# ParBLiSS/kmerhash

Measured on AMD Instinct MI355X. Metric: kmer_inserts_plus_finds_per_sec, higher is better.
Workload: dtype u64

## Files before the change

### kmerhash_amd/csrc/kh_kernels.h

```cpp
#pragma once
#include <hip/hip_runtime.h>
#include <stdint.h>
#include "../../include/kmerhash_amd/kh_hash.h"

#define KH_LB 11
#define KH_L (1u << KH_LB)
#define KH_HS 4096u
#define KH_CHUNK_THREADS 512
#ifndef KH_PART_THREADS
#define KH_PART_THREADS 512
#define KH_PART_MAXPER 4
#endif
#ifndef KH_PART_ITEMS
#define KH_PART_ITEMS 16
#endif
#define KH_PART_TILE (KH_PART_THREADS * KH_PART_ITEMS)
#ifndef KH_PART_STAGE
#define KH_PART_STAGE 4096
#endif
#define KH_NONE 0xFFFFFFFFFFFFFFFFull
#define KH_EMPTY_KEY 0xFFFFFFFFFFFFFFFFull

enum { KHK_RH = 0, KHK_LP = 1 };
enum { KH_FLAG_PROBE_OVERFLOW = 0, KH_FLAG_REGION_OVERFLOW = 1, KH_FLAG_COUNT_OVERFLOW = 2, KH_FLAG_INTERNAL = 3, KH_FLAG_FUSE_INVALID = 4, KH_NFLAGS = 8 };

template <int KIND> __device__ __forceinline__ bool kh_is_empty(uint32_t b) { return KIND == KHK_RH ? (b == 0x00u) : (b == 0x40u); }
template <int KIND> __device__ __forceinline__ bool kh_is_occupied(uint32_t b) { return KIND == KHK_RH ? (b >= 0x80u) : (b < 0x40u); }

struct __align__(16) KhSlot { uint64_t key; uint32_t val; uint32_t info; };
#define KH_INFO_ERASE_MARK 0x100u
struct KhSlots {
  KhSlot* s;
  uint64_t cap;
};
__device__ __forceinline__ uint4 kh_slot_ld(const KhSlot* p) { return *reinterpret_cast<const uint4*>(p); }
__device__ __forceinline__ void kh_slot_st(KhSlot* p, uint64_t key, uint32_t val, uint32_t info) {
  uint4 w; w.x = (uint32_t)key; w.y = (uint32_t)(key >> 32); w.z = val; w.w = info;
  *reinterpret_cast<uint4*>(p) = w;
}
__device__ __forceinline__ uint64_t kh_slot_key(const uint4& w) { return (uint64_t)w.x | ((uint64_t)w.y << 32); }
template <int KIND> __device__ __forceinline__ uint32_t kh_empty_info() { return KIND == KHK_RH ? 0x00u : 0x40u; }

// ... 435 lines not shown
  const KhTile* tiles;
  const uint32_t* ntiles_dev;
  uint32_t ntiles;
  KhSeed seed;
  uint32_t PB;
  uint32_t shift;
  uint32_t nb;
  uint32_t* counts;
  unsigned long long* cursor;
  ulonglong2* orec;
  uint64_t slot;
  uint64_t dump;
  uint32_t* overflow;
  int xcd_swizzle;
  uint64_t slot_in; const unsigned long long* cur_in; uint32_t tps;
};

__device__ __forceinline__ uint32_t kh_part_q(uint64_t h, uint32_t PB) {
  if (PB == 0) return 0;
  uint32_t p = (uint32_t)(h >> KH_LB) & ((1u << PB) - 1u);
  return __brev(p) >> (32 - PB);
}

__device__ __forceinline__ KhTile kh_get_tile(const KhPartParams& P, uint32_t t) {
  if (P.tiles) return P.tiles[t];
  KhTile d;
  d.beg = (uint64_t)t * KH_PART_TILE;
  uint64_t rem = P.n - d.beg;
  d.len = rem < KH_PART_TILE ? (uint32_t)rem : KH_PART_TILE;
  d.seg = 0;
  return d;
}

template <int HASH, bool REC8 = false>
__global__ __launch_bounds__(KH_PART_THREADS) void k_part_hist(KhPartParams P) {
  extern __shared__ __align__(16) uint32_t kh_dyn_smem[];
  uint32_t* hist = kh_dyn_smem;
  const uint32_t tid = threadIdx.x, nb = P.nb;
  const uint32_t ntiles = P.tiles ? *P.ntiles_dev : P.ntiles;
  for (uint32_t i = tid; i < nb; i += KH_PART_THREADS) hist[i] = 0;
  __syncthreads();
  const uint32_t tpb = (ntiles + gridDim.x - 1) / gridDim.x;
  const uint32_t t0 = blockIdx.x * tpb;
  const uint32_t t1 = (t0 + tpb < ntiles) ? t0 + tpb : ntiles;
  uint32_t cur_seg = 0xFFFFFFFFu;
  for (uint32_t t = t0; t < t1; ++t) {
    KhTile d = kh_get_tile(P, t);
    if (d.seg != cur_seg) {
      if (cur_seg != 0xFFFFFFFFu) {
        __syncthreads();
        for (uint32_t i = tid; i < nb; i += KH_PART_THREADS) {
          uint32_t c = hist[i];
// ... 8 lines not shown
                              : *reinterpret_cast<const uint64_t*>(P.kbase + (d.beg + i) * P.kstride);
      uint32_t q = kh_part_q(kh_hash64<HASH>(key, P.seed), P.PB);
      atomicAdd(&hist[(q >> P.shift) & (nb - 1)], 1u);
    }
  }
  __syncthreads();
  if (cur_seg != 0xFFFFFFFFu)
    for (uint32_t i = tid; i < nb; i += KH_PART_THREADS) {
      uint32_t c = hist[i];
      if (c) atomicAdd(&P.counts[(uint64_t)cur_seg * nb + i], c);
    }
}

__device__ __forceinline__ void kh_rec_set(ulonglong2& r, uint64_t key, unsigned long long iv) { r = make_ulonglong2(key, iv); }
__device__ __forceinline__ void kh_rec_set(KhRec12& r, uint64_t key, unsigned long long iv) { r.klo = (uint32_t)key; r.khi = (uint32_t)(key >> 32); r.val = (uint32_t)iv; }
__device__ __forceinline__ void kh_rec_get(const ulonglong2& r, uint64_t& key, unsigned long long& iv) { key = r.x; iv = r.y; }
__device__ __forceinline__ void kh_rec_get(const KhRec12& r, uint64_t& key, unsigned long long& iv) { key = r.klo | ((uint64_t)r.khi << 32); iv = r.val; }
struct KhRec8 { uint64_t key; };
__device__ __forceinline__ void kh_rec_set(KhRec8& r, uint64_t key, unsigned long long) { r.key = key; }
__device__ __forceinline__ void kh_rec_get(const KhRec8& r, uint64_t& key, unsigned long long& iv) { key = r.key; iv = 0; }
template <int RK> struct KhRecOf { typedef ulonglong2 type; };
template <> struct KhRecOf<1> { typedef KhRec12 type; };
template <> struct KhRecOf<2> { typedef KhRec8 type; };
#ifdef KH_PART_OCC3
#define KH_PART_LB(RK) __launch_bounds__(KH_PART_THREADS, (RK) ? 6 : 4)
#define KH_PART_STAGE_OF(RK) ((RK) == 1 ? 3072u : (uint32_t)KH_PART_STAGE)
#else
#define KH_PART_LB(RK) __launch_bounds__(KH_PART_THREADS)
#define KH_PART_STAGE_OF(RK) ((uint32_t)KH_PART_STAGE)
#endif
template <int HASH, int RK>
__global__ KH_PART_LB(RK) void k_part_scatter(KhPartParams P) {
  constexpr bool R12 = RK != 0;
  constexpr uint32_t STAGE = KH_PART_STAGE_OF(RK);
  typedef typename KhRecOf<RK>::type Rec;
  extern __shared__ __align__(16) uint32_t kh_dyn_smem[];
  __shared__ Rec lrec[STAGE];
  __shared__ uint16_t ld[STAGE];
  __shared__ uint32_t wtot[KH_PART_THREADS / 64];
  const uint32_t nb = P.nb;
  uint32_t* hist = kh_dyn_smem;
  uint32_t* loff = kh_dyn_smem + nb;
  unsigned long long* gbase = reinterpret_cast<unsigned long long*>(kh_dyn_smem + 2 * ((nb + 1u) & ~1u));
  const uint32_t tid = threadIdx.x, lane = tid & 63, wid = tid >> 6;
  const uint32_t ntiles = P.tiles ? *P.ntiles_dev : P.ntiles;
  if (blockIdx.x >= ntiles) return;
  uint32_t tile = blockIdx.x;
  if (P.xcd_swizzle && (tile | 63u) < ntiles) {
    const uint32_t x = tile & 7u, j = (tile >> 3) & 7u;
    tile = (tile & ~63u) + x * 8u + j;
  }
  KhTile d;
  uint32_t last;
  unsigned long long fill_end = 0;
  if (P.slot_in) {
    const uint32_t seg = tile / P.tps, k = tile - seg * P.tps;
    fill_end = P.cur_in[seg];
    d.seg = seg; d.beg = (uint64_t)seg * P.slot_in + (uint64_t)k * KH_PART_TILE; d.len = 0;
    const uint64_t room = P.slot_in - (uint64_t)k * KH_PART_TILE;
    last = (room < KH_PART_TILE ? (uint32_t)room : KH_PART_TILE) - 1u;
  } else {
    d = kh_get_tile(P, tile);
    if (d.len == 0) return;
    last = d.len - 1u;
  }
  for (uint32_t i = tid; i < nb; i += KH_PART_THREADS) hist[i] = 0;
  uint64_t key[KH_PART_ITEMS];
  unsigned long long iv[KH_PART_ITEMS];
  uint32_t dr[KH_PART_ITEMS];
  if (P.rec_in) {
    const Rec* src = reinterpret_cast<const Rec*>(P.rec_in) + d.beg;
    Rec rr[KH_PART_ITEMS];
#pragma unroll
    for (int j = 0; j < KH_PART_ITEMS; ++j) { const uint32_t i = tid + j * KH_PART_THREADS; rr[j] = src[i < last ? i : last]; }
#pragma unroll
    for (int j = 0; j < KH_PART_ITEMS; ++j) kh_rec_get(rr[j], key[j], iv[j]);
  } else {
    const char* kb = P.kbase + d.beg * P.kstride;
#pragma unroll
    for (int j = 0; j < KH_PART_ITEMS; ++j) {
      const uint32_t i = tid + j * KH_PART_THREADS, ic = i < last ? i : last;
      key[j] = *reinterpret_cast<const uint64_t*>(kb + (uint64_t)ic * P.kstride);
    }
    if (P.vbase) {
      const char* vb = P.vbase + d.beg * P.vstride;
#pragma unroll
      for (int j = 0; j < KH_PART_ITEMS; ++j) {
        const uint32_t i = tid + j * KH_PART_THREADS, ic = i < last ? i : last;
        iv[j] = *reinterpret_cast<const uint32_t*>(vb + (uint64_t)ic * P.vstride);
      }
    } else {
#pragma unroll
      for (int j = 0; j < KH_PART_ITEMS; ++j) iv[j] = P.vconst;
    }
    if (!R12) {
      const uint64_t pos0 = P.idx_base + d.beg;
#pragma unroll
      for (int j = 0; j < KH_PART_ITEMS; ++j) iv[j] |= (unsigned long long)(pos0 + tid + j * KH_PART_THREADS) << 32;
    }
  }
  if (P.slot_in) {
    const uint64_t sbeg = (uint64_t)d.seg * P.slot_in;
    uint64_t fill = fill_end - sbeg;
    if (fill > P.slot_in) fill = P.slot_in;
    const uint64_t off = d.beg - sbeg;
    if (off == (uint64_t)(P.tps - 1u) * KH_PART_TILE && fill > (uint64_t)P.tps * KH_PART_TILE && tid == 0) *P.overflow = 1u;
    d.len = fill > off ? (fill - off < KH_PART_TILE ? (uint32_t)(fill - off) : KH_PART_TILE) : 0u;
    if (d.len == 0) return;
  }
  __syncthreads();
#pragma unroll
  for (int j = 0; j < KH_PART_ITEMS; ++j) {
    const uint32_t i = tid + j * KH_PART_THREADS;
    const uint32_t q = kh_part_q(kh_hash64<HASH>(key[j], P.seed), P.PB);
    const uint32_t dg = (q >> P.shift) & (nb - 1);
    dr[j] = dg << 16;
    if (i < d.len) dr[j] |= atomicAdd(&hist[dg], 1u);
  }
  __syncthreads();
  const uint32_t per = (nb + KH_PART_THREADS - 1) / KH_PART_THREADS;
  uint32_t mine = 0;
  for (uint32_t k = 0; k < per; ++k) { uint32_t b = tid * per + k; if (b < nb) mine += hist[b]; }
  uint32_t incl = mine;
  for (int off = 1; off < 64; off <<= 1) {
    uint32_t o = __shfl_up(incl, off, 64);
    if (lane >= (uint32_t)off) incl += o;
  }
  if (lane == 63) wtot[wid] = incl;
  __syncthreads();
  uint32_t run = incl - mine;
  for (uint32_t w = 0; w < wid; ++w) run += wtot[w];
  unsigned long long gres[KH_PART_MAXPER];
#pragma unroll
  for (uint32_t k = 0; k < KH_PART_MAXPER; ++k) {
    gres[k] = 0;
    const uint32_t b = tid * per + k;
    if (k < per && b < nb) {
      const uint32_t c = hist[b];
      loff[b] = run;
      run += c;
      if (c) {
        unsigned long long g = atomicAdd(&P.cursor[(uint64_t)d.seg * nb + b], (unsigned long long)c);
        if (P.slot && g + c > ((uint64_t)d.seg * nb + b + 1) * P.slot) { *P.overflow = 1u; g = P.dump + loff[b]; }
        gres[k] = g;
      }
    }
  }
  __syncthreads();
  for (uint32_t r0 = 0; r0 < d.len; r0 += STAGE) {
    if (r0) __syncthreads();
#pragma unroll
    for (int j = 0; j < KH_PART_ITEMS; ++j) {
      uint32_t i = tid + j * KH_PART_THREADS;
      if (i < d.len) {
        const uint32_t dg = dr[j] >> 16;
        const uint32_t s = loff[dg] + (dr[j] & 0xFFFFu) - r0;
        if (s < STAGE) { kh_rec_set(lrec[s], key[j], iv[j]); ld[s] = (uint16_t)dg; }
      }
    }
    if (r0 == 0) {
#pragma unroll
      for (uint32_t k = 0; k < KH_PART_MAXPER; ++k) {
        const uint32_t b = tid * per + k;
        if (k < per && b < nb) gbase[b] = gres[k];
      }
    }
    __syncthreads();
    const uint32_t rl = d.len - r0 < STAGE ? d.len - r0 : STAGE;
    for (uint32_t s = tid; s < rl; s += KH_PART_THREADS) {
      const uint32_t dd = ld[s];
      const uint64_t pos = gbase[dd] + (r0 + s - loff[dd]);
      reinterpret_cast<Rec*>(P.orec)[pos] = lrec[s];
    }
  }
}

#define KH_FULLHIST_THREADS 1024
template <int HASH>
__global__ __launch_bounds__(KH_FULLHIST_THREADS) void k_part_hist_full(const char* __restrict__ kbase, uint32_t kstride, uint64_t n, KhSeed seed,
                                                                         uint32_t PB, uint32_t slice, uint32_t slice_bits,
                                                                         uint32_t* __restrict__ counts ) {
  extern __shared__ __align__(16) uint32_t kh_dyn_smem[];
  const uint32_t lb = PB - slice_bits;
  const uint32_t words = lb ? (1u << (lb - 1)) : 1u;
  const uint32_t lmask = (1u << lb) - 1u;
  for (uint32_t i = threadIdx.x; i < words; i += KH_FULLHIST_THREADS) kh_dyn_smem[i] = 0;
  __syncthreads();
  const uint64_t per = (n + gridDim.x - 1) / gridDim.x;
  const uint64_t b0 = (uint64_t)blockIdx.x * per;
  const uint64_t b1 = b0 + per < n ? b0 + per : n;
  for (uint64_t i0 = b0 + threadIdx.x; i0 < b1; i0 += 8 * KH_FULLHIST_THREADS) {
    uint64_t key[8];
// ... 2806 lines not shown
```

### kmerhash_amd/csrc/kmerhash_amd.hip

```cpp
#include "kh_kernels.h"
#include "kh_kernels_wide.h"
#include "../../include/kmerhash_amd.h"

#include <string>
#include <vector>
#include <cstdio>
#include <cstring>
#include <algorithm>
#include <cmath>
#include <cstdlib>

#include <map>
#include <memory>
#include <mutex>
#include <unordered_map>

#define KH_VERSION_STR "kmerhash_amd 0.1 (gfx950)"

namespace {
struct DevPool {
  std::mutex m;
  std::multimap<size_t, void*> free_;
  std::unordered_map<void*, size_t> size_of;
  size_t cached = 0;
// ... 470 lines not shown
  { kh_status ps = arena_prepare(t, ws_rebuild(n)); if (ps != KH_OK) return ps; }
  return rebuild(t, n, nullptr, nullptr, nullptr, nullptr, 0, false, t->lsize);
}
kh_status do_reserve(kh_table* t, uint64_t n) {
  if (n > t->max_load) return do_rehash(t, static_cast<uint64_t>(static_cast<float>(n) / t->max_lf));
  return KH_OK;
}

struct Partitioned {
  ulonglong2* rec;
  uint64_t* part_off;
  uint32_t PB, nparts;
  ulonglong2* spare;
  uint64_t slot;
  const unsigned long long* cursor;
  uint32_t* overflow;
  int rec12;
};
inline uint64_t slack_slot(double mean, double vf = 1.0) { return (uint64_t)(mean + 7.0 * std::sqrt(mean * vf) + 16.0); }
const bool g_disable_slack = getenv("KH_DISABLE_SLACK_PARTITION") != nullptr;
const int g_xcd_swizzle = getenv("KH_DISABLE_XCD_SWIZZLE") ? 0 : 1;
inline uint64_t part_buffer_records(uint64_t n, uint32_t PB, bool allow_slack, double vf = 1.0) {
  if (!allow_slack || g_disable_slack || PB <= 11 || n < (uint64_t(256) << PB)) return n;
  return (slack_slot((double)n / (double)(uint64_t(1) << PB), vf) << PB) + KH_PART_TILE;
}

kh_status partition_batch(kh_table* t, const char* kbase, uint32_t kstride, const char* vbase, uint32_t vstride,
                          uint32_t vconst, uint64_t n, uint64_t idx_base, uint32_t PB, ulonglong2* tmp, ulonglong2* fin, Partitioned& out,
                          bool allow_slack = false, int rec12 = 0, const SlackShared* shared = nullptr, bool force_slack = false, double vf = 1.0) {
  const uint32_t nparts = 1u << PB;
  out.slot = 0; out.cursor = nullptr; out.overflow = nullptr; out.rec12 = 0;
  if (shared || force_slack || part_buffer_records(n, PB, allow_slack, vf) != n) {
    const uint32_t B1 = (PB + 1) / 2, B2 = PB - B1, nb1 = 1u << B1, nb2 = 1u << B2;
    const uint64_t slot = shared ? shared->slot : slack_slot((double)n / (double)nparts, vf);
    const uint64_t slot1 = shared ? slack_slot((double)n / (double)nb1) : slot * nb2;
    unsigned long long *cur1, *cur2; uint64_t* starts; uint32_t* ovf;
    TAKE(cur1, unsigned long long, nb1);
    if (shared) { cur2 = shared->cur2; starts = shared->starts; ovf = shared->ovf; }
    else { TAKE(cur2, unsigned long long, nparts); TAKE(starts, uint64_t, (size_t)nparts + 1); TAKE(ovf, uint32_t, 1); }
    const double mean1 = (double)n / (double)nb1;
    const uint64_t fill_cap = std::min<uint64_t>(slot1, (uint64_t)(mean1 + 9.0 * std::sqrt(mean1 * vf) + 16.0));
    const uint32_t tps = (uint32_t)((fill_cap + KH_PART_TILE - 1) / KH_PART_TILE);
    const uint32_t max_tiles = nb1 * tps;
    if (shared) hipLaunchKernelGGL(k_init_cursors, dim3((nb1 + 255) / 256), dim3(256), 0, t->stream, cur1, (uint64_t*)nullptr, (uint64_t)nb1, slot1);
    else hipLaunchKernelGGL(k_init_cursors2, dim3((nparts + 256) / 256), dim3(256), 0, t->stream, cur1, (uint64_t)nb1, slot1, cur2, starts, (uint64_t)nparts, slot, ovf);
    KhPartParams P;
    memset(&P, 0, sizeof(P));
    P.idx_base = idx_base;
    P.xcd_swizzle = g_xcd_swizzle;
    P.kbase = kbase; P.kstride = kstride; P.vbase = vbase; P.vstride = vstride; P.vconst = vconst; P.n = n;
    P.ntiles = (uint32_t)((n + KH_PART_TILE - 1) / KH_PART_TILE);
    P.seed = t->seed; P.PB = PB; P.shift = B2; P.nb = nb1; P.cursor = cur1; P.orec = tmp; P.slot = slot1; P.overflow = ovf; P.dump = slot1 * nb1;
    { Launch L(t, "k_part_scatter");
      if (rec12 == 1) { KH_SWITCH_HASH(t->hash, hipLaunchKernelGGL((k_part_scatter<HASH, 1>), dim3(P.ntiles), dim3(KH_PART_THREADS), ((nb1 + 1u) & ~1u) * 8 + nb1 * 8, t->stream, P)); }
      else if (rec12 == 2) { KH_SWITCH_HASH(t->hash, hipLaunchKernelGGL((k_part_scatter<HASH, 2>), dim3(P.ntiles), dim3(KH_PART_THREADS), ((nb1 + 1u) & ~1u) * 8 + nb1 * 8, t->stream, P)); }
      else { KH_SWITCH_HASH(t->hash, hipLaunchKernelGGL((k_part_scatter<HASH, 0>), dim3(P.ntiles), dim3(KH_PART_THREADS), ((nb1 + 1u) & ~1u) * 8 + nb1 * 8, t->stream, P)); } }
    KhPartParams Q = P;
    Q.kbase = nullptr; Q.kstride = 0; Q.vbase = nullptr; Q.vstride = 0; Q.rec_in = tmp;
    Q.tiles = nullptr; Q.ntiles_dev = nullptr; Q.ntiles = max_tiles; Q.slot_in = slot1; Q.cur_in = cur1; Q.tps = tps;
    Q.shift = 0; Q.nb = nb2; Q.cursor = cur2; Q.orec = fin; Q.slot = slot; Q.dump = slot * nparts;
    { Launch L(t, "k_part_scatter");
      if (rec12 == 1) { KH_SWITCH_HASH(t->hash, hipLaunchKernelGGL((k_part_scatter<HASH, 1>), dim3(max_tiles), dim3(KH_PART_THREADS), ((nb2 + 1u) & ~1u) * 8 + nb2 * 8, t->stream, Q)); }
      else if (rec12 == 2) { KH_SWITCH_HASH(t->hash, hipLaunchKernelGGL((k_part_scatter<HASH, 2>), dim3(max_tiles), dim3(KH_PART_THREADS), ((nb2 + 1u) & ~1u) * 8 + nb2 * 8, t->stream, Q)); }
      else { KH_SWITCH_HASH(t->hash, hipLaunchKernelGGL((k_part_scatter<HASH, 0>), dim3(max_tiles), dim3(KH_PART_THREADS), ((nb2 + 1u) & ~1u) * 8 + nb2 * 8, t->stream, Q)); } }
    HIPCHK(hipGetLastError());
    out.rec = fin; out.part_off = starts; out.PB = PB; out.nparts = nparts; out.spare = tmp;
    out.slot = slot; out.cursor = cur2; out.overflow = ovf; out.rec12 = rec12;
    return KH_OK;
  }
  if (rec12 == 1) return fail(t, KH_ERR_HIP, "internal: record kind not available with exact offsets");
  ulonglong2* ar = nullptr; ulonglong2* br = fin;
  const uint32_t B1 = PB <= 11 ? PB : (PB + 1) / 2, B2 = PB - B1;
  const uint32_t nb1 = 1u << B1, nb2 = 1u << B2;
  ar = B2 ? tmp : fin;
  uint32_t* counts1; uint64_t* off1; unsigned long long* cur1;
  TAKE(counts1, uint32_t, nb1); TAKE(off1, uint64_t, nb1 + 1); TAKE(cur1, unsigned long long, nb1);
  KhPartParams P;
  memset(&P, 0, sizeof(P));
  P.idx_base = idx_base;
  P.xcd_swizzle = g_xcd_swizzle;
  P.kbase = kbase; P.kstride = kstride; P.vbase = vbase; P.vstride = vstride; P.vconst = vconst; P.rec_in = nullptr; P.n = n;
  P.tiles = nullptr; P.ntiles_dev = nullptr; P.ntiles = (uint32_t)((n + KH_PART_TILE - 1) / KH_PART_TILE);
  P.seed = t->seed; P.PB = PB; P.shift = B2; P.nb = nb1; P.counts = counts1; P.cursor = cur1;
  P.orec = ar;
  KhTile* tiles = nullptr; uint32_t* ntiles_dev = nullptr; uint32_t* counts2 = nullptr; uint64_t* off2 = nullptr; unsigned long long* cur2 = nullptr;
// ... 82 lines not shown
kh_status insert_finish(kh_table* t, KhSrcSet S, uint64_t n, uint32_t PB, uint64_t cap_u, int mode, uint64_t forced_cap,
                        ulonglong2* spare, uint64_t* n_new_out, uint64_t list_cap = 0);

inline bool fused_build_applies(const kh_table* t, uint64_t cap_u, uint32_t PB) {
  return t->lsize == 0 && cap_u >= 2 * (uint64_t)KH_L && t->max_lf <= 0.9f && PB == log2u(cap_u >> KH_LB) && !g_disable_fused;
}
inline bool nodup_build_applies(const kh_table* t, uint64_t cap_u, uint32_t PB, int mode) {
  return fused_build_applies(t, cap_u, PB) && t->batch_nodup && mode != INS_UPDATE && !getenv("KH_DISABLE_NODUP");
}

kh_status insert_core(kh_table* t, const char* kbase, uint32_t kstride, const char* vbase, uint32_t vstride,
                      uint64_t n, int mode, uint64_t forced_cap, uint64_t* n_new_out) {
  *n_new_out = 0;
  if (n == 0) return KH_OK;
  const uint64_t cap_u = forced_cap ? forced_cap : capacity_after(t, t->cur.cap, t->lsize, n, n, n - 1);
  const uint32_t PB = cap_u > KH_L ? log2u(cap_u >> KH_LB) : 0u;
  if (PB > 22) return fail(t, KH_ERR_UNSUPPORTED, "batch would need more than 2^22 partitions");
  const size_t keep_blk = t->blk, keep_off = t->off;
  int first_attempt = 0;
  bool dup_heavy = false;
  double vf = 1.0;
  if (part_buffer_records(n, PB, true) != n) {
    unsigned long long* sset; uint32_t* dups;
    TAKE(sset, unsigned long long, KH_SAMPLE_SET); TAKE(dups, uint32_t, 1);
    HIPCHK(hipMemsetAsync(sset, 0, sizeof(unsigned long long) * KH_SAMPLE_SET, t->stream));
    HIPCHK(hipMemsetAsync(dups, 0, 4, t->stream));
    { Launch L(t, "k_sample_dups");
      hipLaunchKernelGGL(k_sample_dups, dim3(KH_SAMPLE_N / 256), dim3(256), 0, t->stream, kbase, kstride, n, sset, dups); }
    HIPCHK(hipMemcpyAsync(t->hpin + 31, dups, 4, hipMemcpyDeviceToHost, t->stream));
    HIPCHK(hipStreamSynchronize(t->stream));
    const uint32_t dsample = (uint32_t)t->hpin[31];
    if (dsample >= 1u) {
      dup_heavy = true;
      const double d_ub = (double)dsample + 3.0 * std::sqrt((double)dsample) + 3.0;
      const double f = 1.0 + 2.0 * (double)n * d_ub / ((double)KH_SAMPLE_N * (double)KH_SAMPLE_N);
      const double mean = (double)n / (double)(uint64_t(1) << PB);
      if (!getenv("KH_DISABLE_DUP_SLACK") && (double)slack_slot(mean, f) <= 2.0 * mean) vf = f;
      else first_attempt = 1;
    }
    t->batch_nodup = dsample == 0u;
    t->blk = keep_blk; t->off = keep_off;
  } else first_attempt = 1;
  for (int attempt = first_attempt; attempt < 2; ++attempt) {
    const bool slack = attempt == 0;
    const uint64_t m = part_buffer_records(n, PB, slack, vf);
    if (!slack && attempt == 1) { t->blk = keep_blk; t->off = keep_off; }
    const bool rec12 = slack && t->batch_nodup && nodup_build_applies(t, cap_u, PB, mode);
    const bool rec8 = !rec12 && dup_heavy && mode == INS_PLUS && vbase == nullptr && !getenv("KH_DISABLE_REC8");
    const int kind = rec12 ? 1 : rec8 ? 2 : 0;
// ... 529 lines not shown
    }
    st = launch_find(t, out_pairs ? KH_FIND_PAIRS : KH_FIND_COMPACT, q, n, out_pairs ? nullptr : cv, nullptr, out_pairs ? nullptr : ck,
                     out_pairs ? cp : nullptr, &hits_dev);
    if (st != KH_OK) return st;
    HIPCHK(hipMemcpyAsync(t->hpin, hits_dev, 8, hipMemcpyDeviceToHost, t->stream));
    HIPCHK(hipStreamSynchronize(t->stream));
    hits = t->hpin[0];
    if (host && hits) {
      if (out_pairs) { HIPCHK(hipMemcpyAsync(out_pairs, cp, hits * 16, hipMemcpyDeviceToHost, t->stream)); HIPCHK(hipStreamSynchronize(t->stream)); }
      else { st = copy_compacted(t, hits, ck, cv, out_ckeys, out_cvals); if (st != KH_OK) return st; }
    }
  }
  if (n_found) *n_found = hits;
  return KH_OK;
}

kh_status erase_core(kh_table* t, const void* keys, uint64_t n, kh_mem where, uint64_t* n_erased) {
  *n_erased = 0;
  if (t->ins.active) return refuse_streaming(t);
  if (n == 0) return KH_OK;
  if (!keys) return fail(t, KH_ERR_INVALID, "null keys");
  HIPCHK(hipSetDevice(t->device));
  { kh_status ps = inplace_ok(t, n) ? arena_prepare(t, n * 8 + ws_inplace(t, n))
                                    : arena_prepare(t, n * 8 + 2 * 8 * ((slack_slot((double)n / (double)std::max<uint64_t>(1, t->cur.cap >> KH_LB)) * std::max<uint64_t>(1, t->cur.cap >> KH_LB)) + KH_PART_TILE + n) +
                                                       ws_rebuild(t->cur.cap) + (t->cur.cap > KH_L ? (t->cur.cap >> KH_LB) : 1) * 96 + (n / KH_PART_TILE + 4096) * 16 + (size_t(2) << 20));
    if (ps != KH_OK) return ps; }
  const uint64_t* q;
  kh_status st = stage_in<uint64_t>(t, keys, n, where, &q);
  if (st != KH_OK) return st;
  if (t->kind == KHK_RH && n <= KH_SMALL_N && t->lsize > 0 && !g_disable_small) {
    uint64_t ne = 0; uint32_t done = 0;
    st = small_batch(t, reinterpret_cast<const char*>(q), 8, nullptr, 0, 0, (uint32_t)n, KH_SMALL_ERASE, &ne, &done);
    if (st != KH_OK) return st;
    t->lsize -= ne;
    *n_erased = ne;
    return KH_OK;
  }
  if (inplace_ok(t, n)) {
    KhInplaceParams src;
    memset(&src, 0, sizeof(src));
    src.in_k = q; src.n = n;
    IpResult* res = nullptr;
    st = inplace_passes<KH_IP_ERASE>(t, src, n, &res);
    if (st != KH_OK) return st;
    HIPCHK(hipMemcpyAsync(t->hpin, &res->done, 8, hipMemcpyDeviceToHost, t->stream));
    HIPCHK(hipStreamSynchronize(t->stream));
    t->lsize -= t->hpin[0];
    *n_erased = t->hpin[0];
    return KH_OK;
  }
  const uint32_t PBe = t->cur.cap > KH_L ? log2u(t->cur.cap >> KH_LB) : 0u;
  if (t->kind == KHK_RH && !g_disable_fused_rebuild && !getenv("KH_DISABLE_STREAM_ERASE") && t->cur.cap >= 2 * (uint64_t)KH_L && PBe <= 22 &&
      t->lsize > 0 && t->lsize <= threshold(t->cur.cap, 0.9f) && n <= 0xFFFFFFF0ull) {
    const size_t keep_blk = t->blk, keep_off = t->off;
    const bool slack = PBe > 11 && !g_disable_slack;
    const uint64_t mrec = slack ? (slack_slot((double)n / (double)(uint64_t(1) << PBe)) << PBe) + KH_PART_TILE : n;
    char *a, *b;
    TAKE(a, char, mrec * sizeof(KhRec8)); TAKE(b, char, mrec * sizeof(KhRec8));
    Partitioned R;
    st = partition_batch(t, reinterpret_cast<const char*>(q), 8, nullptr, 0, 0u, n, 0, PBe, reinterpret_cast<ulonglong2*>(a), reinterpret_cast<ulonglong2*>(b), R, slack, 2, nullptr, slack);
    if (st != KH_OK) return st;
    t->part_overflow = R.overflow;
    KhSlots nw;
    st = fresh_slots(t, t->cur.cap, nw);
    if (st != KH_OK) return st;
    KhFusedParams F;
    memset(&F, 0, sizeof(F));
    F.src.rec[0] = R.rec; F.src.off[0] = R.part_off; F.src.n = 1; F.src.merged_off = R.part_off; F.src.slot[0] = R.slot; F.src.cur[0] = R.cursor; F.src.rec12 = 2;
    F.PB = PBe; F.mode = KH_DEDUP_ERASE;
    F.R.Old = narrow(t->cur); F.R.PB = PBe;
    FusedRun run;
    const bool ordered = (R.slot != 0 ? R.slot <= KH_ES_MAXK : n / (uint64_t(1) << PBe) <= KH_ES_MAXK / 2) && !getenv("KH_DISABLE_ORDERED_ERASE");
    { kh_status fs = launch_fused(t, ordered ? 4 : 3, F, nw, PBe, "k_erase_fused", &run); t->part_overflow = nullptr; if (fs != KH_OK) return fs; }
    const uint32_t* ff = reinterpret_cast<const uint32_t*>(reinterpret_cast<const char*>(t->hpin) + 64);
    bool bad = R.overflow && (uint32_t)t->hpin[30];
    for (int i = 0; i < KH_NFLAGS; ++i) bad = bad || ff[i] != 0;
    const uint64_t placed = t->hpin[0];
    if (!bad && placed <= t->lsize) {
      adopt_slots(t, nw);
// ... 16 lines not shown
  HIPCHK(hipStreamSynchronize(t->stream));
  const uint64_t ne = t->hpin[0];
  if (ne && t->kind == KHK_RH) {
    st = rebuild(t, t->cur.cap, nullptr, nullptr, nullptr, nullptr, 0, true, t->lsize - ne);
    if (st != KH_OK) {
      hipLaunchKernelGGL(k_clear_marks, dim3(grid_for(t->cur.cap, 256)), dim3(256), 0, t->stream, narrow(t->cur));
      hipStreamSynchronize(t->stream);
      return st;
    }
  }
  t->lsize -= ne;
  *n_erased = ne;
  return KH_OK;
}

bool valid(const kh_table* t) { return t != nullptr; }
kh_status table_init(kh_table* t, int kind, int hash, uint64_t seed, uint64_t capacity, float min_lf, float max_lf, int device) {
  t->kind = kind; t->hash = hash; t->device = device; t->seed = KhSeed{seed, 0u};
  t->min_lf = min_lf; t->max_lf = max_lf;
  const uint64_t cap = next_pow2(capacity);
  if (alloc_slots(t, cap, t->cur) != KH_OK) return KH_ERR_NOMEM;
  t->hpin = pinned_get();
  if (!t->hpin) { free_slots(t, t->cur); return KH_ERR_NOMEM; }
  if (fill_empty(t, t->cur) != KH_OK || hipStreamSynchronize(t->stream) != hipSuccess) { free_slots(t, t->cur); pinned_put(t->hpin); return KH_ERR_HIP; }
  t->min_load = threshold(cap, min_lf);
  t->max_load = threshold(cap, max_lf);
  return KH_OK;
}
void table_release(kh_table* t) {
  if (!t) return;
  hipSetDevice(t->device);
  hipStreamSynchronize(t->stream);
  for (auto& r : t->recs) { event_put(t->device, r.a); event_put(t->device, r.b); }
  free_slots(t, t->cur); free_slots(t, t->spare);
  for (auto& b : t->blocks) pool_free(t->device, b.p);
  pinned_put(t->hpin);
}

}

extern "C" {

const char* kh_version(void) { return KH_VERSION_STR; }

kh_status kh_release_cached_memory(int device) {
  if (device < 0 || device >= 16) return KH_ERR_INVALID;
  if (hipSetDevice(device) != hipSuccess) return KH_ERR_HIP;
// ... 121 lines not shown
  } else {
    if (t->ins.S.n == KH_MAX_SRC) return fail(t, KH_ERR_UNSUPPORTED, "more than 16 feeds in one streamed insert");
    if (t->ins.S.n == 0 && n >= KH_SAMPLE_N) {
      unsigned long long* sset; uint32_t* dups;
      TAKE(sset, unsigned long long, KH_SAMPLE_SET); TAKE(dups, uint32_t, 1);
      HIPCHK(hipMemsetAsync(sset, 0, sizeof(unsigned long long) * KH_SAMPLE_SET, t->stream));
      HIPCHK(hipMemsetAsync(dups, 0, 4, t->stream));
      { Launch L(t, "k_sample_dups");
        hipLaunchKernelGGL(k_sample_dups, dim3(KH_SAMPLE_N / 256), dim3(256), 0, t->stream, reinterpret_cast<const char*>(dk), 8u, n, sset, dups); }
      HIPCHK(hipMemcpyAsync(t->hpin + 31, dups, 4, hipMemcpyDeviceToHost, t->stream));
      HIPCHK(hipStreamSynchronize(t->stream));
      t->ins.nodup = (uint32_t)t->hpin[31] == 0u;
      t->ins.slack = t->ins.repeatable && (uint32_t)t->hpin[31] == 0u && part_buffer_records(t->ins.n_total, t->ins.PB, true) != t->ins.n_total;
    }
    if (t->ins.S.n == 0 && t->ins.repeatable) {
      const uint64_t nt = t->ins.n_total;
      if (t->ins.slack) {
        const uint32_t nparts = 1u << t->ins.PB;
        t->batch_nodup = t->ins.nodup;
        t->ins.rec12 = nodup_build_applies(t, t->ins.cap_u, t->ins.PB, t->ins.mode);
        t->batch_nodup = false;
        SlackShared& sh = t->ins.sh;
        sh.slot = slack_slot((double)nt / (double)nparts);
        char* f; TAKE(f, char, (sh.slot * nparts + KH_PART_TILE) * (t->ins.rec12 ? sizeof(KhRec12) : sizeof(ulonglong2)));
        t->ins.fin = reinterpret_cast<ulonglong2*>(f);
        TAKE(sh.cur2, unsigned long long, nparts); TAKE(sh.starts, uint64_t, (size_t)nparts + 1); TAKE(sh.ovf, uint32_t, 1);
        HIPCHK(hipMemsetAsync(sh.ovf, 0, 4, t->stream));
        hipLaunchKernelGGL(k_init_cursors, dim3((nparts + 256) / 256), dim3(256), 0, t->stream, sh.cur2, sh.starts, (uint64_t)nparts, sh.slot);
      } else { TAKE(t->ins.tmp, ulonglong2, nt); TAKE(t->ins.fin, ulonglong2, nt); }
    }
    Partitioned R;
    if (t->ins.slack) {
      const uint32_t B1 = (t->ins.PB + 1) / 2, nb1 = 1u << B1;
      const uint64_t slot1 = slack_slot((double)n / (double)nb1);
      char* tm; TAKE(tm, char, (slot1 * nb1 + KH_PART_TILE) * (t->ins.rec12 ? sizeof(KhRec12) : sizeof(ulonglong2)));
      st = partition_batch(t, reinterpret_cast<const char*>(dk), 8, reinterpret_cast<const char*>(dv), 4, t->ins.mode == INS_PLUS ? 1u : 0u,
                           n, t->ins.fed, t->ins.PB, reinterpret_cast<ulonglong2*>(tm), t->ins.fin, R, true, t->ins.rec12, &t->ins.sh);
      if (st != KH_OK) return st;
      t->ins.S.n = 1;
    } else {
      st = partition_batch(t, reinterpret_cast<const char*>(dk), 8, reinterpret_cast<const char*>(dv), 4, t->ins.mode == INS_PLUS ? 1u : 0u,
                           n, t->ins.fed, t->ins.PB, t->ins.tmp, t->ins.fin + t->ins.fed, R);
      if (st != KH_OK) return st;
      t->ins.S.rec[t->ins.S.n] = R.rec; t->ins.S.off[t->ins.S.n] = R.part_off; ++t->ins.S.n;
    }
  }
  t->ins.fed += n;
  if (where == KH_MEM_HOST) HIPCHK(hipStreamSynchronize(t->stream));
  return KH_OK;
}

kh_status kh_insert_end(kh_table* t, uint64_t* n_inserted) {
  if (n_inserted) *n_inserted = 0;
  if (!t) return KH_ERR_INVALID;
  if (!t->ins.active) return fail(t, KH_ERR_INVALID, "kh_insert_end without kh_insert_begin");
  t->ins.active = false;
  if (t->ins.fed != t->ins.n_total) return fail(t, KH_ERR_INVALID, "fewer pairs fed than announced to kh_insert_begin");
  HIPCHK(hipSetDevice(t->device));
  uint64_t nn = 0;
  kh_status st = KH_OK;
  const uint64_t n = t->ins.n_total;
  if (n) {
    if (t->ins.fallback) {
      st = insert_device(t, reinterpret_cast<const char*>(t->ins.stage_k), 8, reinterpret_cast<const char*>(t->ins.stage_v), 4, n, t->ins.mode, &nn);
    } else if (t->ins.slack) {
      const uint32_t nparts = 1u << t->ins.PB;
      const uint64_t list_cap = t->ins.sh.slot * nparts + KH_PART_TILE;
      KhSrcSet S;
      memset(&S, 0, sizeof(S));
      S.rec[0] = t->ins.fin; S.off[0] = t->ins.sh.starts; S.n = 1; S.merged_off = t->ins.sh.starts;
      S.slot[0] = t->ins.sh.slot; S.cur[0] = t->ins.sh.cur2; S.rec12 = t->ins.rec12 ? 1u : 0u;
      char* spare; TAKE(spare, char, list_cap * 16);
      t->part_overflow = t->ins.sh.ovf; t->batch_nodup = t->ins.nodup;
      st = insert_finish(t, S, n, t->ins.PB, t->ins.cap_u, t->ins.mode, 0, reinterpret_cast<ulonglong2*>(spare), &nn, list_cap);
      t->part_overflow = nullptr; t->batch_nodup = false;
      if (st == KH_RETRY_EXACT) {
        if (n_inserted) *n_inserted = 0;
        HIPCHK(hipStreamSynchronize(t->stream));
        t->err = "the speculative partition of this repeatable streamed insert did not hold: feed the same pieces again (kh_insert_begin without KH_INS_REPEATABLE)";
        return KH_ERR_RETRY;
      }
    } else {
      KhSrcSet S = t->ins.S;
      if (S.n == 1) S.merged_off = S.off[0];
      else {
        uint64_t* mo;
        const uint64_t nq1 = (uint64_t(1) << t->ins.PB) + 1;
        TAKE(mo, uint64_t, nq1);
        hipLaunchKernelGGL(k_merge_offsets, dim3((uint32_t)((nq1 + 255) / 256)), dim3(256), 0, t->stream, S, nq1, mo);
        S.merged_off = mo;
// ... 977 lines not shown
```

Baseline: 45.07 billion.

## Use 1024-thread, larger-tile partition scatter for 12-byte records

```diff
diff --git a/kmerhash_amd/csrc/kh_kernels.h b/kmerhash_amd/csrc/kh_kernels.h
--- a/kmerhash_amd/csrc/kh_kernels.h
+++ b/kmerhash_amd/csrc/kh_kernels.h
@@ -7,17 +7,14 @@
 #define KH_L (1u << KH_LB)
 #define KH_HS 4096u
 #define KH_CHUNK_THREADS 512
-#ifndef KH_PART_THREADS
 #define KH_PART_THREADS 512
-#define KH_PART_MAXPER 4
-#endif
-#ifndef KH_PART_ITEMS
 #define KH_PART_ITEMS 16
-#endif
 #define KH_PART_TILE (KH_PART_THREADS * KH_PART_ITEMS)
-#ifndef KH_PART_STAGE
 #define KH_PART_STAGE 4096
-#endif
+#define KH_PART_BIG_THREADS 1024
+#define KH_PART_BIG_STAGE 8192
+#define KH_PART_BIG_TILE (KH_PART_BIG_THREADS * KH_PART_ITEMS)
+#define KH_PART_DUMP KH_PART_BIG_TILE
 #define KH_NONE 0xFFFFFFFFFFFFFFFFull
 #define KH_EMPTY_KEY 0xFFFFFFFFFFFFFFFFull
 
@@ -499,12 +496,12 @@
   return __brev(p) >> (32 - PB);
 }
 
-__device__ __forceinline__ KhTile kh_get_tile(const KhPartParams& P, uint32_t t) {
+__device__ __forceinline__ KhTile kh_get_tile(const KhPartParams& P, uint32_t t, uint32_t tile = KH_PART_TILE) {
   if (P.tiles) return P.tiles[t];
   KhTile d;
-  d.beg = (uint64_t)t * KH_PART_TILE;
+  d.beg = (uint64_t)t * tile;
   uint64_t rem = P.n - d.beg;
-  d.len = rem < KH_PART_TILE ? (uint32_t)rem : KH_PART_TILE;
+  d.len = rem < tile ? (uint32_t)rem : tile;
   d.seg = 0;
   return d;
 }
@@ -559,22 +556,17 @@
 template <int RK> struct KhRecOf { typedef ulonglong2 type; };
 template <> struct KhRecOf<1> { typedef KhRec12 type; };
 template <> struct KhRecOf<2> { typedef KhRec8 type; };
-#ifdef KH_PART_OCC3
-#define KH_PART_LB(RK) __launch_bounds__(KH_PART_THREADS, (RK) ? 6 : 4)
-#define KH_PART_STAGE_OF(RK) ((RK) == 1 ? 3072u : (uint32_t)KH_PART_STAGE)
-#else
-#define KH_PART_LB(RK) __launch_bounds__(KH_PART_THREADS)
-#define KH_PART_STAGE_OF(RK) ((uint32_t)KH_PART_STAGE)
-#endif
-template <int HASH, int RK>
-__global__ KH_PART_LB(RK) void k_part_scatter(KhPartParams P) {
+template <int HASH, int RK, int LANES = KH_PART_THREADS, int ITEMS = KH_PART_ITEMS, int STAGE_N = KH_PART_STAGE>
+__global__ __launch_bounds__(LANES) void k_part_scatter(KhPartParams P) {
   constexpr bool R12 = RK != 0;
-  constexpr uint32_t STAGE = KH_PART_STAGE_OF(RK);
+  constexpr uint32_t STAGE = STAGE_N, TILE = LANES * ITEMS;
+  constexpr uint32_t MAXPER = (2048 + LANES - 1) / LANES;
+  static_assert(TILE <= 65536 && LANES % 64 == 0 && TILE <= KH_PART_DUMP, "rank field of dr[] is 16 bits; the dump area holds one tile");
   typedef typename KhRecOf<RK>::type Rec;
   extern __shared__ __align__(16) uint32_t kh_dyn_smem[];
   __shared__ Rec lrec[STAGE];
   __shared__ uint16_t ld[STAGE];
-  __shared__ uint32_t wtot[KH_PART_THREADS / 64];
+  __shared__ uint32_t wtot[LANES / 64];
   const uint32_t nb = P.nb;
   uint32_t* hist = kh_dyn_smem;
   uint32_t* loff = kh_dyn_smem + nb;
@@ -593,47 +585,47 @@
   if (P.slot_in) {
     const uint32_t seg = tile / P.tps, k = tile - seg * P.tps;
     fill_end = P.cur_in[seg];
-    d.seg = seg; d.beg = (uint64_t)seg * P.slot_in + (uint64_t)k * KH_PART_TILE; d.len = 0;
-    const uint64_t room = P.slot_in - (uint64_t)k * KH_PART_TILE;
-    last = (room < KH_PART_TILE ? (uint32_t)room : KH_PART_TILE) - 1u;
+    d.seg = seg; d.beg = (uint64_t)seg * P.slot_in + (uint64_t)k * TILE; d.len = 0;
+    const uint64_t room = P.slot_in - (uint64_t)k * TILE;
+    last = (room < TILE ? (uint32_t)room : TILE) - 1u;
   } else {
-    d = kh_get_tile(P, tile);
+    d = kh_get_tile(P, tile, TILE);
     if (d.len == 0) return;
     last = d.len - 1u;
   }
-  for (uint32_t i = tid; i < nb; i += KH_PART_THREADS) hist[i] = 0;
-  uint64_t key[KH_PART_ITEMS];
-  unsigned long long iv[KH_PART_ITEMS];
-  uint32_t dr[KH_PART_ITEMS];
+  for (uint32_t i = tid; i < nb; i += LANES) hist[i] = 0;
+  uint64_t key[ITEMS];
+  unsigned long long iv[ITEMS];
+  uint32_t dr[ITEMS];
   if (P.rec_in) {
     const Rec* src = reinterpret_cast<const Rec*>(P.rec_in) + d.beg;
-    Rec rr[KH_PART_ITEMS];
-#pragma unroll
-    for (int j = 0; j < KH_PART_ITEMS; ++j) { const uint32_t i = tid + j * KH_PART_THREADS; rr[j] = src[i < last ? i : last]; }
-#pragma unroll
-    for (int j = 0; j < KH_PART_ITEMS; ++j) kh_rec_get(rr[j], key[j], iv[j]);
+    Rec rr[ITEMS];
+#pragma unroll
+    for (int j = 0; j < ITEMS; ++j) { const uint32_t i = tid + j * LANES; rr[j] = src[i < last ? i : last]; }
+#pragma unroll
+    for (int j = 0; j < ITEMS; ++j) kh_rec_get(rr[j], key[j], iv[j]);
   } else {
     const char* kb = P.kbase + d.beg * P.kstride;
 #pragma unroll
-    for (int j = 0; j < KH_PART_ITEMS; ++j) {
-      const uint32_t i = tid + j * KH_PART_THREADS, ic = i < last ? i : last;
+    for (int j = 0; j < ITEMS; ++j) {
+      const uint32_t i = tid + j * LANES, ic = i < last ? i : last;
       key[j] = *reinterpret_cast<const uint64_t*>(kb + (uint64_t)ic * P.kstride);
     }
     if (P.vbase) {
       const char* vb = P.vbase + d.beg * P.vstride;
 #pragma unroll
-      for (int j = 0; j < KH_PART_ITEMS; ++j) {
-        const uint32_t i = tid + j * KH_PART_THREADS, ic = i < last ? i : last;
+      for (int j = 0; j < ITEMS; ++j) {
+        const uint32_t i = tid + j * LANES, ic = i < last ? i : last;
         iv[j] = *reinterpret_cast<const uint32_t*>(vb + (uint64_t)ic * P.vstride);
       }
     } else {
 #pragma unroll
-      for (int j = 0; j < KH_PART_ITEMS; ++j) iv[j] = P.vconst;
+      for (int j = 0; j < ITEMS; ++j) iv[j] = P.vconst;
     }
     if (!R12) {
       const uint64_t pos0 = P.idx_base + d.beg;
 #pragma unroll
-      for (int j = 0; j < KH_PART_ITEMS; ++j) iv[j] |= (unsigned long long)(pos0 + tid + j * KH_PART_THREADS) << 32;
+      for (int j = 0; j < ITEMS; ++j) iv[j] |= (unsigned long long)(pos0 + tid + j * LANES) << 32;
     }
   }
   if (P.slot_in) {
@@ -641,21 +633,21 @@
     uint64_t fill = fill_end - sbeg;
     if (fill > P.slot_in) fill = P.slot_in;
     const uint64_t off = d.beg - sbeg;
-    if (off == (uint64_t)(P.tps - 1u) * KH_PART_TILE && fill > (uint64_t)P.tps * KH_PART_TILE && tid == 0) *P.overflow = 1u;
-    d.len = fill > off ? (fill - off < KH_PART_TILE ? (uint32_t)(fill - off) : KH_PART_TILE) : 0u;
+    if (off == (uint64_t)(P.tps - 1u) * TILE && fill > (uint64_t)P.tps * TILE && tid == 0) *P.overflow = 1u;
+    d.len = fill > off ? (fill - off < TILE ? (uint32_t)(fill - off) : TILE) : 0u;
     if (d.len == 0) return;
   }
   __syncthreads();
 #pragma unroll
-  for (int j = 0; j < KH_PART_ITEMS; ++j) {
-    const uint32_t i = tid + j * KH_PART_THREADS;
+  for (int j = 0; j < ITEMS; ++j) {
+    const uint32_t i = tid + j * LANES;
     const uint32_t q = kh_part_q(kh_hash64<HASH>(key[j], P.seed), P.PB);
     const uint32_t dg = (q >> P.shift) & (nb - 1);
     dr[j] = dg << 16;
     if (i < d.len) dr[j] |= atomicAdd(&hist[dg], 1u);
   }
   __syncthreads();
-  const uint32_t per = (nb + KH_PART_THREADS - 1) / KH_PART_THREADS;
+  const uint32_t per = (nb + LANES - 1) / LANES;
   uint32_t mine = 0;
   for (uint32_t k = 0; k < per; ++k) { uint32_t b = tid * per + k; if (b < nb) mine += hist[b]; }
   uint32_t incl = mine;
@@ -667,9 +659,9 @@
   __syncthreads();
   uint32_t run = incl - mine;
   for (uint32_t w = 0; w < wid; ++w) run += wtot[w];
-  unsigned long long gres[KH_PART_MAXPER];
-#pragma unroll
-  for (uint32_t k = 0; k < KH_PART_MAXPER; ++k) {
+  unsigned long long gres[MAXPER];
+#pragma unroll
+  for (uint32_t k = 0; k < MAXPER; ++k) {
     gres[k] = 0;
     const uint32_t b = tid * per + k;
     if (k < per && b < nb) {
@@ -687,8 +679,8 @@
   for (uint32_t r0 = 0; r0 < d.len; r0 += STAGE) {
     if (r0) __syncthreads();
 #pragma unroll
-    for (int j = 0; j < KH_PART_ITEMS; ++j) {
-      uint32_t i = tid + j * KH_PART_THREADS;
+    for (int j = 0; j < ITEMS; ++j) {
+      uint32_t i = tid + j * LANES;
       if (i < d.len) {
         const uint32_t dg = dr[j] >> 16;
         const uint32_t s = loff[dg] + (dr[j] & 0xFFFFu) - r0;
@@ -697,14 +689,14 @@
     }
     if (r0 == 0) {
 #pragma unroll
-      for (uint32_t k = 0; k < KH_PART_MAXPER; ++k) {
+      for (uint32_t k = 0; k < MAXPER; ++k) {
         const uint32_t b = tid * per + k;
         if (k < per && b < nb) gbase[b] = gres[k];
       }
     }
     __syncthreads();
     const uint32_t rl = d.len - r0 < STAGE ? d.len - r0 : STAGE;
-    for (uint32_t s = tid; s < rl; s += KH_PART_THREADS) {
+    for (uint32_t s = tid; s < rl; s += LANES) {
       const uint32_t dd = ld[s];
       const uint64_t pos = gbase[dd] + (r0 + s - loff[dd]);
       reinterpret_cast<Rec*>(P.orec)[pos] = lrec[s];
diff --git a/kmerhash_amd/csrc/kmerhash_amd.hip b/kmerhash_amd/csrc/kmerhash_amd.hip
--- a/kmerhash_amd/csrc/kmerhash_amd.hip
+++ b/kmerhash_amd/csrc/kmerhash_amd.hip
@@ -516,7 +516,7 @@
 const int g_xcd_swizzle = getenv("KH_DISABLE_XCD_SWIZZLE") ? 0 : 1;
 inline uint64_t part_buffer_records(uint64_t n, uint32_t PB, bool allow_slack, double vf = 1.0) {
   if (!allow_slack || g_disable_slack || PB <= 11 || n < (uint64_t(256) << PB)) return n;
-  return (slack_slot((double)n / (double)(uint64_t(1) << PB), vf) << PB) + KH_PART_TILE;
+  return (slack_slot((double)n / (double)(uint64_t(1) << PB), vf) << PB) + KH_PART_DUMP;
 }
 
 kh_status partition_batch(kh_table* t, const char* kbase, uint32_t kstride, const char* vbase, uint32_t vstride,
@@ -534,7 +534,8 @@
     else { TAKE(cur2, unsigned long long, nparts); TAKE(starts, uint64_t, (size_t)nparts + 1); TAKE(ovf, uint32_t, 1); }
     const double mean1 = (double)n / (double)nb1;
     const uint64_t fill_cap = std::min<uint64_t>(slot1, (uint64_t)(mean1 + 9.0 * std::sqrt(mean1 * vf) + 16.0));
-    const uint32_t tps = (uint32_t)((fill_cap + KH_PART_TILE - 1) / KH_PART_TILE);
+    const uint32_t tile = rec12 == 1 ? KH_PART_BIG_TILE : KH_PART_TILE;
+    const uint32_t tps = (uint32_t)((fill_cap + tile - 1) / tile);
     const uint32_t max_tiles = nb1 * tps;
     if (shared) hipLaunchKernelGGL(k_init_cursors, dim3((nb1 + 255) / 256), dim3(256), 0, t->stream, cur1, (uint64_t*)nullptr, (uint64_t)nb1, slot1);
     else hipLaunchKernelGGL(k_init_cursors2, dim3((nparts + 256) / 256), dim3(256), 0, t->stream, cur1, (uint64_t)nb1, slot1, cur2, starts, (uint64_t)nparts, slot, ovf);
@@ -543,10 +544,10 @@
     P.idx_base = idx_base;
     P.xcd_swizzle = g_xcd_swizzle;
     P.kbase = kbase; P.kstride = kstride; P.vbase = vbase; P.vstride = vstride; P.vconst = vconst; P.n = n;
-    P.ntiles = (uint32_t)((n + KH_PART_TILE - 1) / KH_PART_TILE);
+    P.ntiles = (uint32_t)((n + tile - 1) / tile);
     P.seed = t->seed; P.PB = PB; P.shift = B2; P.nb = nb1; P.cursor = cur1; P.orec = tmp; P.slot = slot1; P.overflow = ovf; P.dump = slot1 * nb1;
     { Launch L(t, "k_part_scatter");
-      if (rec12 == 1) { KH_SWITCH_HASH(t->hash, hipLaunchKernelGGL((k_part_scatter<HASH, 1>), dim3(P.ntiles), dim3(KH_PART_THREADS), ((nb1 + 1u) & ~1u) * 8 + nb1 * 8, t->stream, P)); }
+      if (rec12 == 1) { KH_SWITCH_HASH(t->hash, hipLaunchKernelGGL((k_part_scatter<HASH, 1, KH_PART_BIG_THREADS, KH_PART_ITEMS, KH_PART_BIG_STAGE>), dim3(P.ntiles), dim3(KH_PART_BIG_THREADS), ((nb1 + 1u) & ~1u) * 8 + nb1 * 8, t->stream, P)); }
       else if (rec12 == 2) { KH_SWITCH_HASH(t->hash, hipLaunchKernelGGL((k_part_scatter<HASH, 2>), dim3(P.ntiles), dim3(KH_PART_THREADS), ((nb1 + 1u) & ~1u) * 8 + nb1 * 8, t->stream, P)); }
       else { KH_SWITCH_HASH(t->hash, hipLaunchKernelGGL((k_part_scatter<HASH, 0>), dim3(P.ntiles), dim3(KH_PART_THREADS), ((nb1 + 1u) & ~1u) * 8 + nb1 * 8, t->stream, P)); } }
     KhPartParams Q = P;
@@ -554,7 +555,7 @@
     Q.tiles = nullptr; Q.ntiles_dev = nullptr; Q.ntiles = max_tiles; Q.slot_in = slot1; Q.cur_in = cur1; Q.tps = tps;
     Q.shift = 0; Q.nb = nb2; Q.cursor = cur2; Q.orec = fin; Q.slot = slot; Q.dump = slot * nparts;
     { Launch L(t, "k_part_scatter");
-      if (rec12 == 1) { KH_SWITCH_HASH(t->hash, hipLaunchKernelGGL((k_part_scatter<HASH, 1>), dim3(max_tiles), dim3(KH_PART_THREADS), ((nb2 + 1u) & ~1u) * 8 + nb2 * 8, t->stream, Q)); }
+      if (rec12 == 1) { KH_SWITCH_HASH(t->hash, hipLaunchKernelGGL((k_part_scatter<HASH, 1, KH_PART_BIG_THREADS, KH_PART_ITEMS, KH_PART_BIG_STAGE>), dim3(max_tiles), dim3(KH_PART_BIG_THREADS), ((nb2 + 1u) & ~1u) * 8 + nb2 * 8, t->stream, Q)); }
       else if (rec12 == 2) { KH_SWITCH_HASH(t->hash, hipLaunchKernelGGL((k_part_scatter<HASH, 2>), dim3(max_tiles), dim3(KH_PART_THREADS), ((nb2 + 1u) & ~1u) * 8 + nb2 * 8, t->stream, Q)); }
       else { KH_SWITCH_HASH(t->hash, hipLaunchKernelGGL((k_part_scatter<HASH, 0>), dim3(max_tiles), dim3(KH_PART_THREADS), ((nb2 + 1u) & ~1u) * 8 + nb2 * 8, t->stream, Q)); } }
     HIPCHK(hipGetLastError());
@@ -683,9 +684,8 @@
   double vf = 1.0;
   if (part_buffer_records(n, PB, true) != n) {
     unsigned long long* sset; uint32_t* dups;
-    TAKE(sset, unsigned long long, KH_SAMPLE_SET); TAKE(dups, uint32_t, 1);
-    HIPCHK(hipMemsetAsync(sset, 0, sizeof(unsigned long long) * KH_SAMPLE_SET, t->stream));
-    HIPCHK(hipMemsetAsync(dups, 0, 4, t->stream));
+    TAKE(sset, unsigned long long, KH_SAMPLE_SET + 1); dups = reinterpret_cast<uint32_t*>(sset + KH_SAMPLE_SET);
+    HIPCHK(hipMemsetAsync(sset, 0, sizeof(unsigned long long) * (KH_SAMPLE_SET + 1), t->stream));
     { Launch L(t, "k_sample_dups");
       hipLaunchKernelGGL(k_sample_dups, dim3(KH_SAMPLE_N / 256), dim3(256), 0, t->stream, kbase, kstride, n, sset, dups); }
     HIPCHK(hipMemcpyAsync(t->hpin + 31, dups, 4, hipMemcpyDeviceToHost, t->stream));
@@ -1261,7 +1261,7 @@
   if (!keys) return fail(t, KH_ERR_INVALID, "null keys");
   HIPCHK(hipSetDevice(t->device));
   { kh_status ps = inplace_ok(t, n) ? arena_prepare(t, n * 8 + ws_inplace(t, n))
-                                    : arena_prepare(t, n * 8 + 2 * 8 * ((slack_slot((double)n / (double)std::max<uint64_t>(1, t->cur.cap >> KH_LB)) * std::max<uint64_t>(1, t->cur.cap >> KH_LB)) + KH_PART_TILE + n) +
+                                    : arena_prepare(t, n * 8 + 2 * 8 * ((slack_slot((double)n / (double)std::max<uint64_t>(1, t->cur.cap >> KH_LB)) * std::max<uint64_t>(1, t->cur.cap >> KH_LB)) + KH_PART_DUMP + n) +
                                                        ws_rebuild(t->cur.cap) + (t->cur.cap > KH_L ? (t->cur.cap >> KH_LB) : 1) * 96 + (n / KH_PART_TILE + 4096) * 16 + (size_t(2) << 20));
     if (ps != KH_OK) return ps; }
   const uint64_t* q;
@@ -1293,7 +1293,7 @@
       t->lsize > 0 && t->lsize <= threshold(t->cur.cap, 0.9f) && n <= 0xFFFFFFF0ull) {
     const size_t keep_blk = t->blk, keep_off = t->off;
     const bool slack = PBe > 11 && !g_disable_slack;
-    const uint64_t mrec = slack ? (slack_slot((double)n / (double)(uint64_t(1) << PBe)) << PBe) + KH_PART_TILE : n;
+    const uint64_t mrec = slack ? (slack_slot((double)n / (double)(uint64_t(1) << PBe)) << PBe) + KH_PART_DUMP : n;
     char *a, *b;
     TAKE(a, char, mrec * sizeof(KhRec8)); TAKE(b, char, mrec * sizeof(KhRec8));
     Partitioned R;
@@ -1356,7 +1356,7 @@
   if (alloc_slots(t, cap, t->cur) != KH_OK) return KH_ERR_NOMEM;
   t->hpin = pinned_get();
   if (!t->hpin) { free_slots(t, t->cur); return KH_ERR_NOMEM; }
-  if (fill_empty(t, t->cur) != KH_OK || hipStreamSynchronize(t->stream) != hipSuccess) { free_slots(t, t->cur); pinned_put(t->hpin); return KH_ERR_HIP; }
+  if (fill_empty(t, t->cur) != KH_OK) { free_slots(t, t->cur); pinned_put(t->hpin); return KH_ERR_HIP; }
   t->min_load = threshold(cap, min_lf);
   t->max_load = threshold(cap, max_lf);
   return KH_OK;
@@ -1524,7 +1524,7 @@
         t->batch_nodup = false;
         SlackShared& sh = t->ins.sh;
         sh.slot = slack_slot((double)nt / (double)nparts);
-        char* f; TAKE(f, char, (sh.slot * nparts + KH_PART_TILE) * (t->ins.rec12 ? sizeof(KhRec12) : sizeof(ulonglong2)));
+        char* f; TAKE(f, char, (sh.slot * nparts + KH_PART_DUMP) * (t->ins.rec12 ? sizeof(KhRec12) : sizeof(ulonglong2)));
         t->ins.fin = reinterpret_cast<ulonglong2*>(f);
         TAKE(sh.cur2, unsigned long long, nparts); TAKE(sh.starts, uint64_t, (size_t)nparts + 1); TAKE(sh.ovf, uint32_t, 1);
         HIPCHK(hipMemsetAsync(sh.ovf, 0, 4, t->stream));
@@ -1535,7 +1535,7 @@
     if (t->ins.slack) {
       const uint32_t B1 = (t->ins.PB + 1) / 2, nb1 = 1u << B1;
       const uint64_t slot1 = slack_slot((double)n / (double)nb1);
-      char* tm; TAKE(tm, char, (slot1 * nb1 + KH_PART_TILE) * (t->ins.rec12 ? sizeof(KhRec12) : sizeof(ulonglong2)));
+      char* tm; TAKE(tm, char, (slot1 * nb1 + KH_PART_DUMP) * (t->ins.rec12 ? sizeof(KhRec12) : sizeof(ulonglong2)));
       st = partition_batch(t, reinterpret_cast<const char*>(dk), 8, reinterpret_cast<const char*>(dv), 4, t->ins.mode == INS_PLUS ? 1u : 0u,
                            n, t->ins.fed, t->ins.PB, reinterpret_cast<ulonglong2*>(tm), t->ins.fin, R, true, t->ins.rec12, &t->ins.sh);
       if (st != KH_OK) return st;
@@ -1567,7 +1567,7 @@
       st = insert_device(t, reinterpret_cast<const char*>(t->ins.stage_k), 8, reinterpret_cast<const char*>(t->ins.stage_v), 4, n, t->ins.mode, &nn);
     } else if (t->ins.slack) {
       const uint32_t nparts = 1u << t->ins.PB;
-      const uint64_t list_cap = t->ins.sh.slot * nparts + KH_PART_TILE;
+      const uint64_t list_cap = t->ins.sh.slot * nparts + KH_PART_DUMP;
       KhSrcSet S;
       memset(&S, 0, sizeof(S));
       S.rec[0] = t->ins.fin; S.off[0] = t->ins.sh.starts; S.n = 1; S.merged_off = t->ins.sh.starts;
```

New measurement: 44.23 billion. -1.9%, worse.
